# kisasexypantera94/hpfw

Hardware: AMD Instinct MI355X
Metric: hashprints/sec (index) + Hamming matches/sec (search), 30 s@44.1 kHz clips (higher is better)
Workload: dtype f32 (transforms, dB) + int8 digits / int64 sums (projection); 1 GPU; configs[1]: 1000 x 30 s synthetic 44.1 kHz PCM16 clips per GPU, hashprint extraction only (CQT + dB + projection + bit pack), inputs resident in HBM; clips_per_gpu=1000, hashprints_per_clip=2320, parallelism=clips sharded over 1 GPU(s), no collective on this path

## Files before the change

### hpfw_amd/csrc/k_forward.hip

```cpp
#include <cstdlib>

#include "kernels.h"

namespace hpfw {

extern __shared__ __align__(16) unsigned char smem_raw[];

typedef int v4i __attribute__((ext_vector_type(4)));
typedef int v16i __attribute__((ext_vector_type(16)));

constexpr int kCqThreads = 256;
constexpr int kCqCols = 128;
constexpr int kCqKSteps = 7;
constexpr int kCqKChunk = 32 * kCqKSteps;
constexpr int kCqTilesPerGroup = 7;
constexpr int kCqPlaneBytes = kCqCols * kCqKChunk;
constexpr int kCqABytes = kCqKSteps * 3 * 1024;
constexpr int kCqLdsBytes = 2 * kCqPlaneBytes + kCqABytes;

__device__ __forceinline__ int cq_slot(int c)
{
    const int l = c & 31;
    return (c & ~31) | (((l >> 2) ^ l) & 1) | (((l >> 3) & 1) << 1) | (((l >> 4) & 1) << 2) | (((l >> 1) & 1) << 3) | ((l & 1) << 4);
}
// ... 338 lines not shown
    cq3_load_samples<LOADW>(a, clip_pcm, col0 + wave * 32, sc, lane, x, [&] { issue_a(0, 0); });
    CQ_STAMP(0);
    const int c = col0 + wave * 32 + nl;
    const bool c_in = c < a.n2;
    const bool vec4 = (a.n2 & 3) == 0;
    static_assert(32 * kCq3Waves == kZBlock, "a workgroup's columns are one block of z");
    float *zblk = z + (int64_t)clip * a.zclip + (int64_t)cb * 2 * a.hq * kZBlock + wave * 32;
    const int rows_live = 2 * a.hq;
    double *corr_lds = reinterpret_cast<double *>(smem_raw + 2 * kCqABytes + kCq3Waves * kCq3ScratchBytes);
    for (int i = tid; i < kCq3CorrRows; i += 64 * kCq3Waves) corr_lds[i] = a.corr[i < rows_live ? i : rows_live - 1];
    for (int mt = 0; mt < a.mt; ++mt) {
        asm volatile("s_waitcnt vmcnt(0) lgkmcnt(0)\n\ts_barrier" ::: "memory");
        CQ_STAMP(1);
        const v4i *wb = reinterpret_cast<const v4i *>(abytes + (mt & 1) * kCqABytes) + lane;
        v16i acc[4];
        const v16i zero = v16i{0};
        auto step = [&](int s) {
            const v4i w0 = wb[(s * 3 + 0) * 64], w1 = wb[(s * 3 + 1) * 64], w2 = wb[(s * 3 + 2) * 64];
            acc[0] = __builtin_amdgcn_mfma_i32_32x32x32_i8(w0, x[s][0], s == 0 ? zero : acc[0], 0, 0, 0);
            acc[1] = __builtin_amdgcn_mfma_i32_32x32x32_i8(w1, x[s][0], s == 0 ? zero : acc[1], 0, 0, 0);
            acc[2] = __builtin_amdgcn_mfma_i32_32x32x32_i8(w2, x[s][0], s == 0 ? zero : acc[2], 0, 0, 0);
            acc[3] = __builtin_amdgcn_mfma_i32_32x32x32_i8(w2, x[s][1], s == 0 ? zero : acc[3], 0, 0, 0);
            acc[1] = __builtin_amdgcn_mfma_i32_32x32x32_i8(w0, x[s][1], acc[1], 0, 0, 0);
            acc[2] = __builtin_amdgcn_mfma_i32_32x32x32_i8(w1, x[s][1], acc[2], 0, 0, 0);
        };
        if (steps == kCqKSteps) {
#pragma unroll
            for (int s = 0; s < kCqKSteps; ++s) step(s);
        } else {
#pragma unroll
            for (int s = 0; s < kCqKSteps; ++s)
                if (s < steps) step(s);
        }
        CQ_STAMP(2);
        CQ_STAMP(3);
        if (mt + 1 < a.mt) issue_a(mt + 1, (mt + 1) & 1);
        asm volatile("" ::: "memory");
        CQ_STAMP(4);
        const int row0 = 32 * mt + 4 * h;
#pragma unroll
        for (int g = 0; g < 4; ++g) {
            float q[4];
#pragma unroll
            for (int e = 0; e < 4; ++e) {
                const int r = 4 * g + e;
                const int lo = acc[0][r] + (acc[1][r] << 8), hi = acc[2][r] + (acc[3][r] << 8);
                q[e] = (float)(__builtin_fma((double)hi, 65536.0, (double)lo) + corr_lds[row0 + 8 * g + e]);
            }
            if (vec4) {
#pragma unroll
                for (int pr = 0; pr < 2; ++pr) {
                    const float send = (lane & 1) ? q[2 * pr] : q[2 * pr + 1];
                    const float got = __builtin_bit_cast(float, __builtin_amdgcn_mov_dpp(__builtin_bit_cast(int, send), 0xB1, 0xF, 0xF, true));
                    if (lane & 1) q[2 * pr] = got; else q[2 * pr + 1] = got;
                }
#pragma unroll
                for (int pr = 0; pr < 2; ++pr) {
                    const float send = (lane & 2) ? q[pr] : q[pr + 2];
                    const float got = __builtin_bit_cast(float, __builtin_amdgcn_mov_dpp(__builtin_bit_cast(int, send), 0x4E, 0xF, 0xF, true));
                    if (lane & 2) q[pr] = got; else q[pr + 2] = got;
                }
                const int row = row0 + 8 * g + (nl & 3);
                const int c4 = col0 + wave * 32 + (nl & ~3);
                if (c4 < a.n2 && row < rows_live) *reinterpret_cast<float4 *>(zblk + row * kZBlock + (nl & ~3)) = float4{q[0], q[1], q[2], q[3]};
            } else {
#pragma unroll
                for (int e = 0; e < 4; ++e) {
                    const int row = row0 + 8 * g + e;
                    if (c_in && row < rows_live) zblk[row * kZBlock + nl] = q[e];
                }
            }
        }
        CQ_STAMP(6);
    }
#ifdef HPFW_COLS_STAMPS
    if (a.stamps && tid == 0) {
        long long *o = a.stamps + (int64_t)blockIdx.x * 8;
#pragma unroll
        for (int k = 0; k < 8; ++k) o[k] = st[k];
    }
#endif
}

#ifdef HPFW_COLS_STAMPS
long long *g_cols_stamps = nullptr;
extern "C" long long *hpfw_debug_cols_stamps() { return g_cols_stamps; }
#endif

constexpr int kFwdThreads = 512;
#ifndef HPFW_ROWS_WAVES
#define HPFW_ROWS_WAVES 6
#endif

template <class Groups, int WAVES>
__global__ __launch_bounds__(kFwdThreads, WAVES) void fwd_rows2_kernel(RowsArgs a, Rows2Out o, const float *__restrict__ z,
                                                                   cf *__restrict__ x)
{
    cf *lds = reinterpret_cast<cf *>(smem_raw);
    const int clip = blockIdx.x, q1 = blockIdx.y;
    rows2_body<Groups>(lds, a, kFwdThreads, z + (int64_t)clip * o.zclip + (int64_t)2 * q1 * o.zrow, q1, o, x + (int64_t)clip * o.n1 * o.q2w);
}

__global__ __launch_bounds__(256) void gather_bins_kernel(CqPlanDev cp, const cf *__restrict__ x, cf *__restrict__ out)
{
    const int clip = blockIdx.y;
    const XsView v = cp.view(x, clip);
    for (int i = blockIdx.x * 256 + threadIdx.x; i < cp.nk; i += gridDim.x * 256) out[(int64_t)clip * cp.nk + i] = v(cp.kmin + i);
}

template <int LOADW>
static void launch_cols_q_t(ColsQArgs a, const int16_t *d_pcm, int64_t clip_samples, dim3 grid, float *d_z, hipStream_t s)
{
    static PerDeviceOnce attr_set;
    if (attr_set.need()) {
        (void)hipFuncSetAttribute(reinterpret_cast<const void *>(fwd_cols_q_kernel<LOADW, true>), hipFuncAttributeMaxDynamicSharedMemorySize, kCqLdsBytes);
        (void)hipFuncSetAttribute(reinterpret_cast<const void *>(fwd_cols_q_kernel<LOADW, false>), hipFuncAttributeMaxDynamicSharedMemorySize, kCqLdsBytes);
        attr_set.mark();
    }
    if (a.ks <= kCqKSteps && !(a.variant & 1)) {
        a.n_clips = grid.x;
        constexpr int kWaves = 4;
        const int ncb = (a.n2 + 32 * kWaves - 1) / (32 * kWaves);
        hipLaunchKernelGGL((fwd_cols_q3_kernel<LOADW, kWaves>), dim3(8 * ((grid.x * ncb + 7) / 8)), dim3(64 * kWaves), cq3_lds_bytes(kWaves), s,
                           a, d_pcm, clip_samples, d_z);
        return;
    }
    if (a.n1 <= 255)
        hipLaunchKernelGGL((fwd_cols_q_kernel<LOADW, true>), grid, dim3(kCqThreads), kCqLdsBytes, s, a, d_pcm, clip_samples, d_z);
    else
        hipLaunchKernelGGL((fwd_cols_q_kernel<LOADW, false>), grid, dim3(kCqThreads), kCqLdsBytes, s, a, d_pcm, clip_samples, d_z);
}

void launch_fwd_cols_q(const ColsQArgs &a_in, const int16_t *d_pcm, int64_t clip_samples, int n_clips, float *d_z, hipStream_t s)
{
    if (n_clips <= 0) return;
    ColsQArgs a = a_in;
#ifdef HPFW_COLS_STAMPS
    static long long *d_stamps = nullptr;
    if (!d_stamps) (void)hipMalloc(&d_stamps, (size_t)64 * 1024 * 1024);
    a.stamps = d_stamps;
    g_cols_stamps = d_stamps;
#endif
    dim3 grid(n_clips, (a.n2 + kCqCols - 1) / kCqCols, (a.mt + kCqTilesPerGroup - 1) / kCqTilesPerGroup);
    const uintptr_t addr = reinterpret_cast<uintptr_t>(d_pcm);
    if (a.n2 % 4 == 0 && a.n2 >= 4 && addr % 8 == 0 && clip_samples % 4 == 0)
        launch_cols_q_t<4>(a, d_pcm, clip_samples, grid, d_z, s);
    else if (a.n2 % 2 == 0 && addr % 4 == 0 && clip_samples % 2 == 0)
        launch_cols_q_t<2>(a, d_pcm, clip_samples, grid, d_z, s);
    else
        launch_cols_q_t<1>(a, d_pcm, clip_samples, grid, d_z, s);
}

size_t fwd_rows_lds_bytes(const RowsArgs &a) { return (size_t)a.n2 * sizeof(cf); }

template <class Groups, int WAVES>
static void launch_rows2_t(const RowsArgs &a, const Rows2Out &o, const float *d_z, int n_clips, cf *d_x, hipStream_t s)
{
    static PerDeviceOnce attr_set;
    if (attr_set.need()) {
        (void)hipFuncSetAttribute(reinterpret_cast<const void *>(fwd_rows2_kernel<Groups, WAVES>),
                                  hipFuncAttributeMaxDynamicSharedMemorySize, 160 * 1024);
        attr_set.mark();
    }
    dim3 grid(n_clips, o.hq);
    hipLaunchKernelGGL((fwd_rows2_kernel<Groups, WAVES>), grid, dim3(kFwdThreads), fwd_rows_lds_bytes(a), s, a, o, d_z, d_x);
}

void launch_fwd_rows2(const RowsArgs &a, const Rows2Out &o, const float *d_z, int n_clips, cf *d_x, hipStream_t s)
{
    if (n_clips <= 0) return;
    if (Groups6300::matches_plan(a) && Groups6300::min_threads(a.n2) <= kFwdThreads)
        launch_rows2_t<Groups6300, HPFW_ROWS_WAVES>(a, o, d_z, n_clips, d_x, s);
    else
        launch_rows2_t<RuntimeGroups, 4>(a, o, d_z, n_clips, d_x, s);
}

void launch_gather_bins(const CqPlanDev &cp, const cf *d_x, int n_clips, cf *d_out, hipStream_t s)
{
    if (n_clips <= 0) return;
    hipLaunchKernelGGL(gather_bins_kernel, dim3((cp.nk + 255) / 256 < 64 ? (cp.nk + 255) / 256 : 64, n_clips), dim3(256), 0, s, cp, d_x, d_out);
}

}
```

### hpfw_amd/csrc/kernels.h

```cpp
#pragma once
#include <cmath>
#include <cstdint>
#include <vector>
#include <atomic>
#include <hip/hip_runtime.h>
#include <stdint.h>

#include "device_math.h"
#include "fft_lds.h"
#include "fft_rows.h"

namespace hpfw {

struct PerDeviceOnce {
    std::atomic<uint64_t> done{0};
    static uint64_t bit()
    {
        int dev = 0;
        (void)hipGetDevice(&dev);
        return 1ull << (dev & 63);
    }
    bool need() const { return !(done.load(std::memory_order_acquire) & bit()); }
    void mark() { done.fetch_or(bit(), std::memory_order_release); }
};


constexpr int kBins = 121;
constexpr int kCtx = 20;
constexpr int kLag = 80;
constexpr int kFilters = 64;
constexpr int kFrame = kBins * kCtx;

constexpr int kZBlock = 128;
inline long long z_floats_per_clip(int hq, int n2) { return (long long)((n2 + kZBlock - 1) / kZBlock) * 2 * hq * kZBlock; }

struct ColsQArgs {
    int n1, n2, hq;
    int mt, ks;
    const void *image;
    const double *corr;
    long long *stamps;
    int n_clips;
    int variant;
    long long zclip;
};

#ifndef HPFW_XS_BATCH
#define HPFW_XS_BATCH 4
#endif
constexpr int kXsBatch = HPFW_XS_BATCH;
struct XsView {
    const cf *base;
    int n1, w, q0;
    unsigned long long magic;
    HPFW_DEVICE_MEMBER cf operator()(int k) const
    {
        if (n1 == 1) return base[k - q0];
        const int q2 = (int)(((unsigned long long)(unsigned)k * magic) >> 40);
        return base[(int64_t)(k - q2 * n1) * w + (q2 - q0)];
    }
};
struct XsBand {
    XsView v;
    int start;
    HPFW_DEVICE_MEMBER cf operator()(int i) const { return v(start + i); }
    template <class F>
    HPFW_DEVICE_MEMBER void for_each(int tid, int nthreads, int lg, const cf *__restrict__ g, F f) const
    {
        for (int i0 = tid; i0 < lg; i0 += kXsBatch * nthreads) {
            cf xv[kXsBatch], gv[kXsBatch];
#pragma unroll
            for (int u = 0; u < kXsBatch; ++u) {
                const int i = i0 + u * nthreads;
                const int ic = i < lg ? i : lg - 1;
                xv[u] = v(start + ic);
                gv[u] = g[ic];
            }
#pragma unroll
            for (int u = 0; u < kXsBatch; ++u) {
                const int i = i0 + u * nthreads;
                if (i < lg) f(i, c_mul(xv[u], gv[u]));
            }
        }
    }
};
struct XsBandRows {
    const cf *base;
    int n1, w, q0;
    int start, q2a, nq2;
    unsigned magic;
    template <class F>
    HPFW_DEVICE_MEMBER void for_each(int tid, int nthreads, int lg, const cf *__restrict__ g2, F f) const
    {
        const int total = n1 * nq2;
        for (int t0 = tid; t0 < total; t0 += kXsBatch * nthreads) {
            cf xv[kXsBatch], gv[kXsBatch];
            int ii[kXsBatch];
#pragma unroll
            for (int u = 0; u < kXsBatch; ++u) {
                const int t = t0 + u * nthreads;
                const int tc = t < total ? t : total - 1;
                const int q1 = nq2 == 1 ? tc : (int)(((unsigned long long)(unsigned)tc * magic) >> 32);
                const int tq = tc - q1 * nq2;
                const int i = q1 + n1 * (q2a + tq) - start;
                ii[u] = (t < total && i >= 0 && i < lg) ? i : -1;
                xv[u] = base[(int64_t)q1 * w + (q2a - q0 + tq)];
                gv[u] = g2[tc];
            }
#pragma unroll
            for (int u = 0; u < kXsBatch; ++u)
                if (ii[u] >= 0) f(ii[u], c_mul(xv[u], gv[u]));
        }
    }
};

struct BzArgs {
    int n1, n2, n2pad;
    int kmin, kmax;
    int a;
    int n_tiles1;
    int k1lo, k1n;
    int n_tiles2;
    int nt2;
    const float *wp;
    const cf *tl;
    const cf *bhat;
// ... 167 lines not shown
```

### hpfw_amd/csrc/plan.cpp

```cpp
#include "plan.h"
#include "trig_d.h"

#include <algorithm>
#include <atomic>
#include <cmath>
#include <cstring>
#include <map>
#include <memory>
#include <mutex>
#include <thread>

namespace hpfw {

namespace {
constexpr double kSampleRate = 44100.0;
constexpr double kMinFreq = 130.81;
constexpr double kMaxFreq = 4186.01;
constexpr int kBpo = 24;
constexpr int kMinWindow = 96;
constexpr int kDown = 3;
constexpr int kBins = 121;
constexpr int kCtx = 20;
constexpr int kLag = 80;
constexpr int64_t kN2Max = 6826;
// ... 309 lines not shown
    }
    const int64_t n2 = p.bluestein ? 6300 : n / n1;
    std::vector<int> tmp;
    std::vector<int> desc;
    if (!make_radix_list(n2, desc) || (!p.bluestein && !make_radix_list(n1, tmp))) {
        why = "clip length has a prime factor other than 2, 3, 5, 7";
        return false;
    }
    for (size_t lo = 0, hi = desc.size(); lo < hi;) {
        p.radix.push_back(desc[lo++]);
        if (lo < hi) p.radix.push_back(desc[--hi]);
    }
    if (n1 > 8192) {
        why = "clip too long";
        return false;
    }
    p.n1 = (int)n1;
    p.n2 = (int)n2;
    p.h = (int)(n2 / 2 + 1);
    p.k1lo = (int)(kmin / n2);
    p.k1hi = (int)((kmax - 1) / n2);
    if (geometry_only) return true;
    p.tw_n2 = twiddle_table(n2);
    p.tw_n1 = twiddle_table(n1);
    for (size_t i = 0; i < p.radix.size();) {
        if (i + 1 < p.radix.size() && p.radix[i] * p.radix[i + 1] <= 36) {
            p.groups.push_back({p.radix[i], p.radix[i + 1]});
            i += 2;
        } else {
            p.groups.push_back({p.radix[i], 1});
            i += 1;
        }
    }
    if (p.groups.size() > 12) {
        why = "too many radix passes";
        return false;
    }
    {
        int64_t len = n2;
        for (const auto &g : p.groups) {
            p.rows_gtw_off.push_back((int)p.rows_gtw.size());
            append_group_twiddles(p.tw_n2, n2, len, g.first, g.second, p.rows_gtw);
            len /= g.first * g.second;
        }
    }
    if (!p.bluestein) {
        const int64_t hq = n1 / 2 + 1;
        p.hq = (int)hq;
        p.q2lo = (int)(kmin / n1);
        p.q2w = (int)((kmax - 1) / n1) - p.q2lo + 1;
        p.cols_mt = (int)((2 * hq + 31) / 32);
        p.cols_ks = (int)((n1 + 31) / 32);
        p.wq.resize((size_t)2 * n1);
        for (int64_t m = 0; m < n1; ++m) {
            double c, s;
            twiddle_d(m, n1, c, s);
            p.wq[(size_t)(2 * m)] = (int32_t)std::rint(c * 4194304.0);
            p.wq[(size_t)(2 * m + 1)] = (int32_t)std::rint(s * 4194304.0);
        }
        p.cols_corr.assign((size_t)2 * hq, 0.0);
        for (int64_t q1 = 0; q1 < hq; ++q1) {
            int64_t sr = 0, si = 0;
            for (int64_t k1 = 0; k1 < n1; ++k1) {
                sr += p.wq[(size_t)(2 * ((q1 * k1) % n1))];
                si += p.wq[(size_t)(2 * ((q1 * k1) % n1) + 1)];
            }
            p.cols_corr[(size_t)(2 * q1)] = (double)(128 * sr);
            p.cols_corr[(size_t)(2 * q1 + 1)] = (double)(128 * si);
        }
        p.cols_image.assign((size_t)p.cols_mt * p.cols_ks * 3 * 1024, 0);
        parallel_rows(p.cols_mt, [&](int64_t mt) {
            for (int64_t ks = 0; ks < p.cols_ks; ++ks)
                for (int l = 0; l < 64; ++l)
                    for (int e = 0; e < 16; ++e) {
                        const int64_t row = 32 * mt + (l & 31), k1 = 32 * ks + 16 * (l >> 5) + e, q1 = row >> 1;
                        if (q1 >= hq || k1 >= n1) continue;
                        const int w = p.wq[(size_t)(2 * ((q1 * k1) % n1) + (row & 1))];
                        const int d0 = ((w + 128) & 255) - 128, w1 = (w - d0) >> 8, d1 = ((w1 + 128) & 255) - 128, d2 = (w1 - d1) >> 8;
                        const int d[3] = {d0, d1, d2};
                        for (int i = 0; i < 3; ++i)
                            p.cols_image[((((size_t)mt * p.cols_ks + ks) * 3 + i) * 64 + l) * 16 + e] = (int8_t)d[i];
                    }
        });
        const int64_t nq = (n2 + 3) / 4;
        p.ts_seed.resize((size_t)(hq * nq));
        p.ts_step.resize((size_t)(hq * 4));
        parallel_rows(hq, [&](int64_t q1) {
            for (int64_t m = 0; m < nq; ++m) {
                const HostCf t = twiddle_f((q1 * 4 * m) % n, n);
                p.ts_seed[(size_t)(q1 * nq + m)] = {std::ldexp(t.r, -37), std::ldexp(t.i, -37)};
            }
            p.ts_step[(size_t)(q1 * 4)] = {1.0f, 0.0f};
            for (int e = 1; e < 4; ++e) p.ts_step[(size_t)(q1 * 4 + e)] = twiddle_f((q1 * e) % n, n);
        });
    }
    p.pos_n2.resize((size_t)n2);
    for (int64_t k = 0; k < n2; ++k) p.pos_n2[(size_t)k] = (int)digit_pos(k, n2, p.radix);
    {
        const int r1 = p.groups.back().first, r2 = p.groups.back().second, len = r1 * r2;
        const int nb = (int)(n2 / len);
        p.kb_last.assign((size_t)nb, -1);
        for (int k = 0; k < nb; ++k) p.kb_last[(size_t)(p.pos_n2[(size_t)k] / len)] = k;
        for (int b = 0; b < nb; ++b)
            for (int s = 0; s < r1; ++s)
                for (int s2 = 0; s2 < r2; ++s2)
                    if (p.kb_last[(size_t)b] < 0 ||
                        p.pos_n2[(size_t)(p.kb_last[(size_t)b] + nb * (s + r1 * s2))] != len * b + s * r2 + s2) {
                        why = "internal: last-group output map";
                        return false;
                    }
    }
    p.g_off.assign(kBins, 0);
    int64_t goff = 0;
    for (int j = 0; j < kBins; ++j) {
        const int64_t need = p.lg[j] + p.c - 1;
        const int64_t ps = chirpz_length(need);
        if (ps > (1 << 19)) {
            why = "clip too long: chirp-z length above 2^19";
            return false;
        }
        p.psize[j] = (int)ps;
        size_t k = 0;
        for (; k < p.classes.size(); ++k)
            if (p.classes[k].p == ps) break;
        if (k == p.classes.size()) {
            BluesteinClass bc;
            bc.p = (int)ps;
            p.classes.push_back(std::move(bc));
        }
        p.classes[k].bands.push_back(j);
        p.g_off[j] = goff;
        goff += p.lg[j];
    }
    std::atomic<bool> bad_class{false};
    parallel_rows((int64_t)p.classes.size(), [&](int64_t ci) {
        BluesteinClass &bc = p.classes[(size_t)ci];
        const int64_t ps = bc.p;
        make_radix_list(ps, bc.radix);
        bc.tw = twiddle_table(ps);
        {
            auto next_radix = [](int64_t len) { return len % 4 == 0 ? 4 : (len % 3 == 0 ? 3 : 2); };
            int64_t len = ps;
            while (ps > 16384 && len > 8192) {
                len /= 4;
                ++bc.outer;
            }
            bc.len0 = (int)len;
            int g = 0;
            for (;;) {
                const int r1 = next_radix(len);
                const int r2 = len / r1 > 1 ? next_radix(len / r1) : 1;
                const int64_t rest = len / (r1 * r2);
                if (rest == 1) {
                    std::vector<HostCf> tmp;
                    append_group_twiddles(bc.tw, ps, len, r1, r2, tmp);
                    bc.mid_off = (int)bc.gtw.size();
                    for (int e = 0; e < (r1 - 1) * r2; ++e) bc.gtw.push_back(tmp[(size_t)e]);
                    break;
                }
                if (g >= 4) {
                    bad_class = true;
                    return;
                }
                bc.goff[g++] = (int)bc.gtw.size();
                append_group_twiddles(bc.tw, ps, len, r1, r2, bc.gtw);
                len /= r1 * r2;
// ... 195 lines not shown
```

### hpfw_amd/csrc/plan.h

```cpp
#pragma once
#include <cstdint>
#include <string>
#include <utility>
#include <vector>

namespace hpfw {

struct HostCf {
    float r, i;
};

struct BluesteinClass {
    int p = 0;
    std::vector<int> radix;
    std::vector<HostCf> tw;
    std::vector<HostCf> gtw;
    int goff[4] = {0, 0, 0, 0};
    int mid_off = 0;
    std::vector<HostCf> vrev;
    std::vector<int> bands;
    int len0 = 0, outer = 0;
};

struct HostPlan {
    int64_t n = 0;
    int n1 = 0, n2 = 0, h = 0;
    int kmin = 0, kmax = 0, k1lo = 0, k1hi = 0;
    int m = 0, c = 0, n_frames = 0, n_hp = 0;
    std::vector<int> radix;
    std::vector<std::pair<int, int>> groups;
    std::vector<HostCf> rows_gtw;
    std::vector<int> rows_gtw_off;
    std::vector<HostCf> tw_n2, tw_n1;
    std::vector<HostCf> tw_big;
    int hq = 0;
    int q2lo = 0, q2w = 0;
    int cols_mt = 0, cols_ks = 0;
    std::vector<int32_t> wq;
    std::vector<int8_t> cols_image;
    std::vector<double> cols_corr;
    std::vector<HostCf> ts_seed;
    std::vector<HostCf> ts_step;
    std::vector<int> pos_n2;
    std::vector<int> kb_last;
    int start[121], lg[121], psize[121];
    std::vector<int64_t> g_off;
    int64_t g_total = 0, big_m = 0;
    std::vector<HostCf> g;
    std::vector<BluesteinClass> classes;
    bool bluestein = false;
    int64_t bz_l = 0;
};

enum : unsigned {
    kConvHannPeriodic = 1u,
    kConvLgHalfEven = 2u,
    kConvFloatGeometry = 4u,
    kConvNoIfftScale = 8u,
    kConvAll = 15u
};
struct PlanSerial {
    PlanSerial();
    ~PlanSerial();
    bool before;
};
bool build_plan(int64_t n_samples, HostPlan &out, std::string &why, bool geometry_only = false,
                bool force_bluestein = false, unsigned conventions = 0, bool host_windows = true);
inline double cq_window_scale(unsigned conventions, int64_t big_m, int psize)
{
    return 1.0 / (((conventions & kConvNoIfftScale) ? 1.0 : (double)big_m) * (double)psize);
}
inline int64_t cq_hann_den(unsigned conventions, int64_t lg) { return (conventions & kConvHannPeriodic) ? lg : lg - 1; }

bool build_frame_transform(int n2, HostPlan &out, std::string &why);
void mel_tables(std::vector<float> &window, std::vector<float> &cpack);

void twiddle_d(int64_t m, int64_t n, double &re, double &im);
int64_t digit_pos(int64_t k, int64_t n, const std::vector<int> &radix);
bool make_radix_list(int64_t n, std::vector<int> &radix);
void append_group_twiddles(const std::vector<HostCf> &tw, int64_t n, int64_t len, int r1, int r2,
                           std::vector<HostCf> &out);

}
```

### hpfw_amd/csrc/plans.hip

```cpp
#include "handle.h"

struct PlanTiming {
    double host_wait = 0, host_build = 0, upload = 0, device_tables = 0, alloc = 0, evict = 0, total = 0;
    long plans = 0, copies = 0;
    size_t copied = 0;
};

namespace {
thread_local size_t g_uploaded = 0;

hpfw::RadixList to_radix(const std::vector<int> &r)
{
    hpfw::RadixList rl;
    std::memset(&rl, 0, sizeof(rl));
    rl.n = (int)r.size();
    for (size_t i = 0; i < r.size(); ++i) rl.r[i] = r[i];
    return rl;
}

DevBuf pool_take(hpfw_gpu *h, size_t bytes);
void pool_give(hpfw_gpu *h, DevBuf b);
void pool_release(hpfw_gpu *h);

constexpr size_t kPlanChunk = (size_t)4 << 20;
// ... 212 lines not shown
    std::memset(&bz, 0, sizeof(bz));
    if (p.bluestein) {
        PlanTimer t_dev(&PlanTiming::device_tables);
        bz.n1 = p.n1;
        bz.n2 = p.n2;
        bz.n2pad = (p.n2 + 31) / 32 * 32;
        bz.kmin = p.kmin;
        bz.kmax = p.kmax;
        bz.a = p.n1 / 16;
        bz.n_tiles1 = (bz.a + 15) / 16;
        bz.k1lo = p.kmin / p.n2;
        bz.k1n = (p.kmax - 1) / p.n2 - bz.k1lo + 1;
        {
            const int need = (2 * bz.k1n + 31) / 32;
            bz.nt2 = need < 3 ? need : 3;
            bz.n_tiles2 = (need + bz.nt2 - 1) / bz.nt2 * bz.nt2;
        }
        const cf *d_tw_n1 = nullptr;
        struct PoolTmp {
            hpfw_gpu *h;
            std::vector<DevBuf> v;
            ~PoolTmp() { for (DevBuf &b : v) pool_give(h, std::move(b)); }
            void *take(size_t bytes)
            {
                DevBuf b = pool_take(h, (bytes + 65535) / 65536 * 65536);
                if (!b) return nullptr;
                v.push_back(std::move(b));
                return v.back().get();
            }
        } tmp{h, {}};
        {
            void *d = tmp.take(p.tw_n1.size() * sizeof(cf));
            if (!d) return fail(HPFW_E_HIP, "out of device memory for the tables of a clip length");
            HIP_TRY(plan_h2d(h, d, p.tw_n1.data(), p.tw_n1.size() * sizeof(cf)));
            d_tw_n1 = static_cast<const cf *>(d);
        }
        {
            const size_t bytes[3] = {(size_t)bz.a * bz.n_tiles1 * 64 * sizeof(float), (size_t)bz.a * 16 * 64 * sizeof(float),
                                     (size_t)p.n1 * bz.n_tiles2 * 64 * sizeof(float)};
            const float **slot[3] = {&bz.apack1, &bz.apack3, &bz.apack2};
            for (int i = 0; i < 3; ++i) {
                void *d = nullptr;
                if ((rc = plan_alloc(dp.get(), bytes[i], &d))) return rc;
                g_uploaded += bytes[i];
                *slot[i] = static_cast<const float *>(d);
            }
            if ((rc = plan_flush(dp.get()))) return rc;
            hpfw::launch_bz_pack_stages(bz, d_tw_n1, const_cast<float *>(bz.apack1), const_cast<float *>(bz.apack3), h->cache.plan_stream.get());
            hpfw::launch_bz_pack_coefficients(p.n1, bz.k1lo, bz.k1n, d_tw_n1, bz.n_tiles2, const_cast<float *>(bz.apack2), h->cache.plan_stream.get());
        }
        const size_t big_l = (size_t)p.n1 * p.n2, plane = hpfw::bz_plane_bytes(bz, 1);
        {
            const size_t bytes[4] = {big_l * sizeof(cf), big_l * sizeof(cf), big_l * sizeof(cf), (size_t)(p.kmax - p.kmin) * sizeof(cf)};
            const void **slot[4] = {reinterpret_cast<const void **>(&bz.wp), reinterpret_cast<const void **>(&bz.tl),
                                    reinterpret_cast<const void **>(&bz.bhat), reinterpret_cast<const void **>(&bz.wk)};
            for (int i = 0; i < 4; ++i) {
                void *d = nullptr;
                if ((rc = plan_alloc(dp.get(), bytes[i], &d))) return rc;
                g_uploaded += bytes[i];
                *slot[i] = d;
            }
        }
        void *scratch = tmp.take(big_l * 8 + plane);
        if (!scratch) return fail(HPFW_E_HIP, "out of device memory for the tables of a clip length");
        hpfw::launch_bz_make_tables(ra, bz, n, static_cast<float *>(scratch), static_cast<float *>(scratch) + 2 * big_l, h->cache.plan_stream.get());
        const hipError_t launched = hipGetLastError();
        if (launched != hipSuccess) return fail(HPFW_E_HIP, std::string("chirp-z tables: ") + hipGetErrorString(launched));
    }
    hpfw::ColsQArgs &ca = dp->cols;
    std::memset(&ca, 0, sizeof(ca));
    dp->rows_out = hpfw::Rows2Out{p.n1, p.hq, p.q2lo, p.q2w, nullptr, nullptr, (p.n2 + 3) / 4, 5 ,
                                  (long long)2 * p.hq * hpfw::kZBlock, hpfw::kZBlock, hpfw::z_floats_per_clip(p.hq, p.n2)};
    static_assert(hpfw::kZBlock == 128, "Rows2Out::zshift4 above");
    if (!p.bluestein) {
        ca.n1 = p.n1;
        ca.n2 = p.n2;
        ca.hq = p.hq;
        ca.mt = p.cols_mt;
        ca.ks = p.cols_ks;
        ca.zclip = hpfw::z_floats_per_clip(p.hq, p.n2);
        const int8_t *img = nullptr;
        if ((rc = upload(p.cols_image, &img, dp.get()))) return rc;
        ca.image = img;
        if ((rc = upload(p.cols_corr, &ca.corr, dp.get()))) return rc;
        if ((rc = upload(p.ts_seed, reinterpret_cast<const hpfw::HostCf **>(&dp->rows_out.seed), dp.get()))) return rc;
        if ((rc = upload(p.ts_step, reinterpret_cast<const hpfw::HostCf **>(&dp->rows_out.step), dp.get()))) return rc;
    }
    hpfw::CqPlanDev &c = dp->cq;
    c.kmin = p.kmin;
    c.nk = p.kmax - p.kmin;
    c.c = p.c;
    if (p.bluestein) {
        c.xn1 = 1;
        c.xw = 0;
        c.xq0 = p.kmin;
        c.xclip = c.nk;
        c.xmagic = 0;
    } else {
        c.xn1 = p.n1;
        c.xw = p.q2w;
        c.xq0 = p.q2lo;
        c.xclip = (int64_t)p.n1 * p.q2w;
        c.xmagic = ((1ull << 40) + (unsigned long long)p.n1 - 1) / (unsigned long long)p.n1;
    }
    std::vector<int> start(p.start, p.start + 121), lg(p.lg, p.lg + 121);
    if ((rc = upload(start, &c.start, dp.get()))) return rc;
    if ((rc = upload(lg, &c.lg, dp.get()))) return rc;
    if ((rc = upload(p.g_off, &c.g_off, dp.get()))) return rc;
    {
        void *d = nullptr;
        if ((rc = plan_alloc(dp.get(), (size_t)std::max<int64_t>(p.g_total, 1) * sizeof(cf), &d))) return rc;
        g_uploaded += (size_t)p.g_total * sizeof(cf);
        c.g = static_cast<const cf *>(d);
    }
    int g2_max_entries = 0;
    c.g2 = nullptr;
    c.g2_off = nullptr;
    c.q2a = c.nq2 = nullptr;
    c.nq2_magic = nullptr;
    c.rows_min = 4;
    if (!p.bluestein) {
        std::vector<int> q2a(121), nq2(121);
        std::vector<unsigned> magic(121);
        std::vector<int64_t> g2_off(121);
        int64_t total = 0;
        for (int j = 0; j < 121; ++j) {
            q2a[j] = p.start[j] / p.n1;
            nq2[j] = (p.start[j] + p.lg[j] - 1) / p.n1 - q2a[j] + 1;
            magic[j] = nq2[j] >= 2 ? (unsigned)(((1ull << 32) + (unsigned)nq2[j] - 1) / (unsigned)nq2[j]) : 0u;
            g2_off[j] = total;
            total += (int64_t)p.n1 * nq2[j];
        }
        for (int j = 0; j < 121; ++j) g2_max_entries = std::max(g2_max_entries, p.n1 * nq2[j]);
        {
            void *d = nullptr;
            if ((rc = plan_alloc(dp.get(), (size_t)std::max<int64_t>(total, 1) * sizeof(cf), &d))) return rc;
            g_uploaded += (size_t)total * sizeof(cf);
            c.g2 = static_cast<const cf *>(d);
        }
        if ((rc = upload(g2_off, &c.g2_off, dp.get()))) return rc;
        if ((rc = upload(q2a, &c.q2a, dp.get()))) return rc;
        if ((rc = upload(nq2, &c.nq2, dp.get()))) return rc;
        if ((rc = upload(magic, &c.nq2_magic, dp.get()))) return rc;
    }
    for (const hpfw::BluesteinClass &bc : p.classes) {
        hpfw::CqClassDev cd;
        cd.p = bc.p;
        cd.n_bands = (int)bc.bands.size();
        cd.radix = to_radix(bc.radix);
        if ((rc = upload(bc.tw, reinterpret_cast<const hpfw::HostCf **>(&cd.tw), dp.get()))) return rc;
        if ((rc = upload(bc.gtw, reinterpret_cast<const hpfw::HostCf **>(&cd.gtw.tab), dp.get()))) return rc;
        for (int g = 0; g < 4; ++g) cd.gtw.off[g] = bc.goff[g];
        cd.gtw.mid_off = bc.mid_off;
        if ((rc = upload(bc.vrev, reinterpret_cast<const hpfw::HostCf **>(&cd.vrev), dp.get()))) return rc;
        if ((rc = upload(bc.bands, &cd.band, dp.get()))) return rc;
        cd.len0 = bc.len0;
        cd.outer = bc.outer;
        dp->cls.push_back(cd);
    }
    if ((size_t)p.n2 * sizeof(cf) > 150 * 1024) return fail(HPFW_E_UNSUPPORTED, "n2 exceeds the LDS");
    {
        hpfw::HostPlan &hp = dp->hp;
        std::vector<hpfw::HostCf>().swap(hp.rows_gtw);
        std::vector<hpfw::HostCf>().swap(hp.tw_n2);
        std::vector<hpfw::HostCf>().swap(hp.tw_n1);
        std::vector<hpfw::HostCf>().swap(hp.ts_seed);
        std::vector<int8_t>().swap(hp.cols_image);
        std::vector<hpfw::HostCf>().swap(hp.g);
        for (hpfw::BluesteinClass &bc : hp.classes) {
            std::vector<hpfw::HostCf>().swap(bc.tw);
            std::vector<hpfw::HostCf>().swap(bc.gtw);
            std::vector<hpfw::HostCf>().swap(bc.vrev);
        }
    }
    dp->bytes = g_uploaded;
    dp->last_use = ++h->cache.plan_clock;
    size_t budget = (size_t)16 << 30;
    if (const char *e = std::getenv("HPFW_PLAN_CACHE_GB")) budget = (size_t)(std::max(0.0, std::atof(e)) * 1073741824.0);
    if (h->cache.plan_bytes + dp->bytes > budget && !h->cache.plans.empty()) {
        PlanTimer t(&PlanTiming::evict);
        size_t goal = budget;
        while (h->cache.plan_bytes + dp->bytes > goal && !h->cache.plans.empty()) {
            auto lru = h->cache.plans.begin();
            for (auto q = h->cache.plans.begin(); q != h->cache.plans.end(); ++q)
                if (q->second->last_use < lru->second->last_use) lru = q;
            if (lru->second->last_use > h->cache.idle_clock) {
                HIP_TRY(hipDeviceSynchronize());
                h->cache.idle_clock = h->cache.plan_clock;
                goal = budget - budget / 4;
            }
            h->cache.plan_bytes -= lru->second->bytes;
            {
                std::scoped_lock lock(h->cache.host_mtx);
                h->cache.host_seen.erase(lru->first);
            }
            h->cache.plans.erase(lru);
        }
    }
    if ((rc = plan_flush(dp.get()))) return rc;
    std::vector<char>().swap(dp->stage);
    {
        PlanTimer t(&PlanTiming::device_tables);
        hpfw::CqWindowBands wb;
        int lg_max = 0;
        for (int j = 0; j < 121; ++j) {
            wb.scale[j] = hpfw::cq_window_scale(h->conventions, p.big_m, p.psize[j]);
            wb.hann_den[j] = (int)hpfw::cq_hann_den(h->conventions, p.lg[j]);
            lg_max = std::max(lg_max, p.lg[j]);
        }
        hpfw::launch_cq_windows(c, wb, p.big_m, lg_max, const_cast<cf *>(c.g), h->cache.plan_stream.get());
        if (c.g2) hpfw::launch_cq_windows_rows(c, p.n1, g2_max_entries, const_cast<cf *>(c.g2), h->cache.plan_stream.get());
        const hipError_t launched = hipGetLastError();
        if (launched != hipSuccess) return fail(HPFW_E_HIP, std::string("constant-Q window tables: ") + hipGetErrorString(launched));
    }
    HIP_TRY(hipEventRecord(h->cache.plan_ev.get(), h->cache.plan_stream.get()));
    h->cache.plan_ev_pending = true;
    h->cache.plan_bytes += dp->bytes;
    *out = dp.get();
    h->cache.plans[n] = std::move(dp);
    return 0;
}

hipError_t init_plans(hpfw_gpu *h)
{
    if (std::getenv("HPFW_PLAN_TIMING")) h->cache.plan_timing = std::make_unique<PlanTiming>();
    const hipError_t e = h->cache.plan_ev.create();
    return e != hipSuccess ? e : h->cache.plan_stream.create();
}

void clear_plans(hpfw_gpu *h)
{
    h->cache.plans.clear();
    h->cache.plan_bytes = 0;
    std::unique_lock<std::mutex> lock(h->cache.host_mtx);
    h->cache.host_cv.wait(lock, [&] {
        for (auto &kv : h->cache.host_ready)
            if (!kv.second) return false;
        return true;
    });
    h->cache.host_ready.clear();
    h->cache.host_seen.clear();
}

hpfw_gpu::PlanCache::PlanCache() = default;
hpfw_gpu::PlanCache::~PlanCache()
{
    if (!plan_timing || !plan_timing->plans) return;
    const PlanTiming &t = *plan_timing;
    std::fprintf(stderr, "hpfw plan timing: %ld lengths, %.1f ms in get_plan = %.3f ms each: wait for the host half %.3f, host build %.3f, "
                         "uploads %.3f (%ld copies, %.2f MB per length), device tables (incl. their uploads) %.3f, device memory %.3f, "
// ... 103 lines not shown
```

Measured before the change: 247.9 million hashprints/s.

## Add symmetry-folded int8 MFMA column DFT kernel using half-period twiddle structure

Result: faster. 263.2 million hashprints/s, median of 6 (+6.2%).

```diff
diff --git a/hpfw_amd/csrc/k_forward.hip b/hpfw_amd/csrc/k_forward.hip
--- a/hpfw_amd/csrc/k_forward.hip
+++ b/hpfw_amd/csrc/k_forward.hip
@@ -444,6 +444,262 @@
 #endif
 }
 
+constexpr int kCq4Steps = 2;
+constexpr int kCq4ABytes = 2 * kCq4Steps * 3 * 1024;
+constexpr int kCq4ScratchBytes = 2 * 4 * 32 * 16;
+constexpr int cq4_lds_bytes(int waves) { return 2 * kCq4ABytes + waves * kCq4ScratchBytes + kCq3CorrRows * 8; }
+
+__device__ __forceinline__ int cq4_slot(int c)
+{
+    return ((c >> 2) & 1) | (((c >> 3) & 1) << 1) | ((((c >> 4) ^ (c >> 1)) & 1) << 2) | ((c & 1) << 3) | (((c >> 1) & 1) << 4);
+}
+
+__device__ __forceinline__ void cq4_store_pair(unsigned char *sc, int c, int rq, unsigned r0, unsigned r1, unsigned r2, unsigned r3)
+{
+    const unsigned x01 = __builtin_amdgcn_perm(r1, r0, 0x05010400u), x23 = __builtin_amdgcn_perm(r3, r2, 0x05010400u);
+    const unsigned y01 = __builtin_amdgcn_perm(r1, r0, 0x07030602u), y23 = __builtin_amdgcn_perm(r3, r2, 0x07030602u);
+    const int a0 = (rq >> 2) * 512 + cq4_slot(c) * 16 + 4 * (rq & 3), a1 = (rq >> 2) * 512 + cq4_slot(c + 1) * 16 + 4 * (rq & 3);
+    *reinterpret_cast<unsigned *>(sc + a0) = __builtin_amdgcn_perm(x23, x01, 0x05040100u);
+    *reinterpret_cast<unsigned *>(sc + 2048 + a0) = __builtin_amdgcn_perm(x23, x01, 0x07060302u);
+    *reinterpret_cast<unsigned *>(sc + a1) = __builtin_amdgcn_perm(y23, y01, 0x05040100u);
+    *reinterpret_cast<unsigned *>(sc + 2048 + a1) = __builtin_amdgcn_perm(y23, y01, 0x07060302u);
+}
+
+template <int LOADW, class F>
+__device__ __forceinline__ void cq4_load_samples(const ColsQArgs &a, const int16_t *__restrict__ clip_pcm, int cw0,
+                                                 unsigned char *sc, int lane, v4i (&x)[2 * kCq4Steps][2][2], F issued)
+{
+    const int cg = lane & 7, quad = lane >> 3;
+    const int row_last = a.n1 - 1, last = a.n2 - 1;
+    const int gc = cw0 + 4 * cg;
+    const char *base = reinterpret_cast<const char *>(clip_pcm);
+    const unsigned pitch = 2u * (unsigned)a.n2;
+    unsigned cb[4];
+    if (LOADW == 4) {
+        cb[0] = 2u * (unsigned)(gc + 3 <= last ? gc : last - 3);
+    } else if (LOADW == 2) {
+        cb[0] = 2u * (unsigned)(gc + 1 <= last ? gc : last - 1);
+        cb[1] = 2u * (unsigned)(gc + 3 <= last ? gc + 2 : last - 1);
+    } else {
+#pragma unroll
+        for (int e = 0; e < 4; ++e) cb[e] = 2u * (unsigned)(gc + e <= last ? gc + e : last);
+    }
+    constexpr int kItems = 2 * kCq4Steps;
+    constexpr int kBatch = LOADW == 4 ? kItems : 1;
+    const int rd0 = (lane >> 4) * 512 + cq4_slot(lane & 15) * 16, rd1 = (lane >> 4) * 512 + cq4_slot(16 + (lane & 15)) * 16;
+#pragma unroll
+    for (int i0 = 0; i0 < kItems; i0 += kBatch) {
+    unsigned r[kBatch][8][2];
+#pragma unroll
+    for (int ib = 0; ib < kBatch; ++ib) {
+        const int par = (i0 + ib) / kCq4Steps, s = (i0 + ib) % kCq4Steps;
+#pragma unroll
+        for (int i = 0; i < 8; ++i) {
+            int row = 2 * (64 * s + 32 * (i >> 2) + 4 * quad + (i & 3)) + par;
+            if (row > row_last) row = row_last;
+            const unsigned ro = (unsigned)row * pitch;
+            if (LOADW == 4) {
+                const uint2 v = *reinterpret_cast<const uint2 *>(base + (ro + cb[0]));
+                r[ib][i][0] = v.x;
+                r[ib][i][1] = v.y;
+            } else if (LOADW == 2) {
+                r[ib][i][0] = *reinterpret_cast<const unsigned *>(base + (ro + cb[0]));
+                r[ib][i][1] = *reinterpret_cast<const unsigned *>(base + (ro + cb[1]));
+            } else {
+                r[ib][i][0] = (unsigned)*reinterpret_cast<const unsigned short *>(base + (ro + cb[0])) |
+                              ((unsigned)*reinterpret_cast<const unsigned short *>(base + (ro + cb[1])) << 16);
+                r[ib][i][1] = (unsigned)*reinterpret_cast<const unsigned short *>(base + (ro + cb[2])) |
+                              ((unsigned)*reinterpret_cast<const unsigned short *>(base + (ro + cb[3])) << 16);
+            }
+        }
+    }
+    if (i0 == 0) issued();
+#pragma unroll
+    for (int ib = 0; ib < kBatch; ++ib) {
+#pragma unroll
+        for (int i = 0; i < 8; ++i) {
+            r[ib][i][0] ^= 0x00800080u;
+            r[ib][i][1] ^= 0x00800080u;
+        }
+#pragma unroll
+        for (int hf = 0; hf < 2; ++hf) {
+            cq4_store_pair(sc, 4 * cg, 8 * hf + quad, r[ib][4 * hf][0], r[ib][4 * hf + 1][0], r[ib][4 * hf + 2][0], r[ib][4 * hf + 3][0]);
+            cq4_store_pair(sc, 4 * cg + 2, 8 * hf + quad, r[ib][4 * hf][1], r[ib][4 * hf + 1][1], r[ib][4 * hf + 2][1], r[ib][4 * hf + 3][1]);
+        }
+        asm volatile("s_waitcnt lgkmcnt(0)" ::: "memory");
+        x[i0 + ib][0][0] = *reinterpret_cast<const v4i *>(sc + rd0);
+        x[i0 + ib][0][1] = *reinterpret_cast<const v4i *>(sc + 2048 + rd0);
+        x[i0 + ib][1][0] = *reinterpret_cast<const v4i *>(sc + rd1);
+        x[i0 + ib][1][1] = *reinterpret_cast<const v4i *>(sc + 2048 + rd1);
+        asm volatile("s_waitcnt lgkmcnt(0)" ::: "memory");
+    }
+    }
+}
+
+__device__ __forceinline__ void cq4_quad_transpose(float (&q)[4], int lane)
+{
+#pragma unroll
+    for (int pr = 0; pr < 2; ++pr) {
+        const float send = (lane & 1) ? q[2 * pr] : q[2 * pr + 1];
+        const float got = __builtin_bit_cast(float, __builtin_amdgcn_mov_dpp(__builtin_bit_cast(int, send), 0xB1, 0xF, 0xF, true));
+        if (lane & 1) q[2 * pr] = got; else q[2 * pr + 1] = got;
+    }
+#pragma unroll
+    for (int pr = 0; pr < 2; ++pr) {
+        const float send = (lane & 2) ? q[pr] : q[pr + 2];
+        const float got = __builtin_bit_cast(float, __builtin_amdgcn_mov_dpp(__builtin_bit_cast(int, send), 0x4E, 0xF, 0xF, true));
+        if (lane & 2) q[pr] = got; else q[pr + 2] = got;
+    }
+}
+
+template <int LOADW, int kCq4Waves>
+__global__ __launch_bounds__(64 * kCq4Waves, 3) void fwd_cols_q4_kernel(ColsQArgs a, const int16_t *__restrict__ pcm, int64_t clip_samples,
+                                                                    float *__restrict__ z)
+{
+    constexpr int kCq4Cols = 32 * kCq4Waves;
+    unsigned char *abytes = smem_raw;
+    const int tid = threadIdx.x, lane = tid & 63, wave = tid >> 6;
+    unsigned char *sc = smem_raw + 2 * kCq4ABytes + wave * kCq4ScratchBytes;
+    const int ncb = (a.n2 + kCq4Cols - 1) / kCq4Cols;
+    const unsigned per_xcd = (gridDim.x + 7) / 8;
+    const unsigned t = (blockIdx.x & 7) * per_xcd + (blockIdx.x >> 3);
+    if (t >= (unsigned)(a.n_clips * ncb)) return;
+    const int cb = t % ncb, clip = t / ncb;
+    const int col0 = cb * kCq4Cols;
+    const int16_t *clip_pcm = pcm + (int64_t)clip * clip_samples;
+    const v4i *image = static_cast<const v4i *>(a.image2);
+    const int ks2 = a.ks2, pieces = 3 * 2 * ks2;
+    auto issue_a = [&](int mt, int buf) {
+        const v4i *src = image + (int64_t)mt * pieces * 64 + lane;
+#pragma unroll
+        for (int e = 0; e < (2 * kCq4Steps * 3 + kCq4Waves - 1) / kCq4Waves; ++e) {
+            const int p = wave + kCq4Waves * e;
+            if (p < pieces)
+                __builtin_amdgcn_global_load_lds((const __attribute__((address_space(1))) void *)(src + p * 64),
+                                                 (__attribute__((address_space(3))) void *)(abytes + buf * kCq4ABytes + p * 1024),
+                                                 16, 0, 0);
+        }
+    };
+#ifdef HPFW_COLS_STAMPS
+    long long st[8] = {0, 0, 0, 0, 0, 0, 0, 0};
+    long long tprev = __builtin_amdgcn_s_memtime();
+    auto stamp = [&](int k) {
+        const long long t = __builtin_amdgcn_s_memtime();
+        st[k] += t - tprev;
+        tprev = t;
+    };
+#endif
+    v4i x[2 * kCq4Steps][2][2];
+    cq4_load_samples<LOADW>(a, clip_pcm, col0 + wave * 32, sc, lane, x, [&] { issue_a(0, 0); });
+    CQ_STAMP(0);
+    const int u = lane >> 4, nl = lane & 15;
+    const int hh = a.n1 >> 1, q1_last = hh >> 1;
+    const bool vec4 = (a.n2 & 3) == 0;
+    static_assert(32 * kCq4Waves == kZBlock, "a workgroup's columns are one block of z");
+    float *zblk = z + (int64_t)clip * a.zclip + (int64_t)cb * 2 * a.hq * kZBlock + wave * 32;
+    const int rows_live = 2 * a.hq;
+    double *corr_lds = reinterpret_cast<double *>(smem_raw + 2 * kCq4ABytes + kCq4Waves * kCq4ScratchBytes);
+    for (int i = tid; i < kCq3CorrRows; i += 64 * kCq4Waves) corr_lds[i] = a.corr[i < rows_live ? i : rows_live - 1];
+    for (int mt = 0; mt < a.mt2; ++mt) {
+        asm volatile("s_waitcnt vmcnt(0) lgkmcnt(0)\n\ts_barrier" ::: "memory");
+        CQ_STAMP(1);
+        const v4i *wb = reinterpret_cast<const v4i *>(abytes + (mt & 1) * kCq4ABytes) + lane;
+        const v4i zero = v4i{0, 0, 0, 0};
+        v4i lo[2][2], hi[2][2];
+#pragma unroll
+        for (int par = 0; par < 2; ++par) {
+            v4i acc[4][2];
+#pragma unroll
+            for (int s = 0; s < kCq4Steps; ++s) {
+                if (s == 0 || s < ks2) {
+                    const v4i *w = wb + (par * ks2 + s) * 3 * 64;
+                    const v4i w0 = w[0], w1 = w[64], w2 = w[128];
+                    const v4i(&xs)[2][2] = x[par * kCq4Steps + s];
+#pragma unroll
+                    for (int ct = 0; ct < 2; ++ct) {
+                        acc[0][ct] = __builtin_amdgcn_mfma_i32_16x16x64_i8(w0, xs[ct][0], s == 0 ? zero : acc[0][ct], 0, 0, 0);
+                        acc[1][ct] = __builtin_amdgcn_mfma_i32_16x16x64_i8(w1, xs[ct][0], s == 0 ? zero : acc[1][ct], 0, 0, 0);
+                        acc[2][ct] = __builtin_amdgcn_mfma_i32_16x16x64_i8(w2, xs[ct][0], s == 0 ? zero : acc[2][ct], 0, 0, 0);
+                        acc[3][ct] = __builtin_amdgcn_mfma_i32_16x16x64_i8(w2, xs[ct][1], s == 0 ? zero : acc[3][ct], 0, 0, 0);
+                    }
+#pragma unroll
+                    for (int ct = 0; ct < 2; ++ct) {
+                        acc[1][ct] = __builtin_amdgcn_mfma_i32_16x16x64_i8(w0, xs[ct][1], acc[1][ct], 0, 0, 0);
+                        acc[2][ct] = __builtin_amdgcn_mfma_i32_16x16x64_i8(w1, xs[ct][1], acc[2][ct], 0, 0, 0);
+                    }
+                }
+            }
+#pragma unroll
+            for (int ct = 0; ct < 2; ++ct) {
+                lo[par][ct] = acc[0][ct] + (acc[1][ct] << 8);
+                hi[par][ct] = acc[2][ct] + (acc[3][ct] << 8);
+            }
+        }
+        CQ_STAMP(2);
+        if (mt + 1 < a.mt2) issue_a(mt + 1, (mt + 1) & 1);
+        asm volatile("" ::: "memory");
+        CQ_STAMP(4);
+        const int q1a = 8 * mt + 2 * u;
+        const double *cp = corr_lds + 16 * mt + 4 * u;
+        const double *cm0 = corr_lds + 2 * max(hh - q1a, 0), *cm1 = corr_lds + 2 * max(hh - q1a - 1, 0);
+        float gp[2][4], gm[2][4];
+#pragma unroll
+        for (int ct = 0; ct < 2; ++ct)
+#pragma unroll
+            for (int r = 0; r < 4; ++r) {
+                const int el = lo[0][ct][r], eh = hi[0][ct][r], ol = lo[1][ct][r], oh = hi[1][ct][r];
+                gp[ct][r] = (float)(__builtin_fma((double)(eh + oh), 65536.0, (double)(el + ol)) + cp[r]);
+                const int ml = (r & 1) ? ol - el : el - ol, mh = (r & 1) ? oh - eh : eh - oh;
+                gm[ct][r] = (float)(__builtin_fma((double)mh, 65536.0, (double)ml) + (r < 2 ? cm0 : cm1)[r & 1]);
+            }
+        if (vec4) {
+            const int j = lane & 3, col = 16 * (u >> 1) + (nl & ~3);
+            const bool c_ok = col0 + wave * 32 + col < a.n2;
+#pragma unroll
+            for (int sgn = 0; sgn < 2; ++sgn) {
+                float(&g)[2][4] = sgn ? gm : gp;
+                cq4_quad_transpose(g[0], lane);
+                cq4_quad_transpose(g[1], lane);
+                float sa[4], sb[4];
+#pragma unroll
+                for (int e = 0; e < 4; ++e) {
+                    const auto sw = __builtin_amdgcn_permlane32_swap(__builtin_bit_cast(unsigned, g[0][e]), __builtin_bit_cast(unsigned, g[1][e]), false, false);
+                    sa[e] = __builtin_bit_cast(float, (unsigned)sw[0]);
+                    sb[e] = __builtin_bit_cast(float, (unsigned)sw[1]);
+                }
+#pragma unroll
+                for (int half = 0; half < 2; ++half) {
+                    const int tr = 8 * half + 4 * (u & 1) + j, q1 = 8 * mt + (tr >> 1);
+                    const int row = sgn ? 2 * (hh - q1) + (tr & 1) : 16 * mt + tr;
+                    const bool live = q1 <= q1_last && (!sgn || 2 * q1 < hh);
+                    const float(&s4)[4] = half ? sb : sa;
+                    if (c_ok && live) *reinterpret_cast<float4 *>(zblk + row * kZBlock + col) = float4{s4[0], s4[1], s4[2], s4[3]};
+                }
+            }
+        } else {
+            const int c = col0 + wave * 32 + nl;
+#pragma unroll
+            for (int ct = 0; ct < 2; ++ct)
+#pragma unroll
+                for (int r = 0; r < 4; ++r) {
+                    const int q1 = q1a + (r >> 1);
+                    if (c + 16 * ct < a.n2 && q1 <= q1_last) {
+                        zblk[(2 * q1 + (r & 1)) * kZBlock + 16 * ct + nl] = gp[ct][r];
+                        if (2 * q1 < hh) zblk[(2 * (hh - q1) + (r & 1)) * kZBlock + 16 * ct + nl] = gm[ct][r];
+                    }
+                }
+        }
+        CQ_STAMP(6);
+    }
+#ifdef HPFW_COLS_STAMPS
+    if (a.stamps && tid == 0) {
+        long long *o = a.stamps + (int64_t)blockIdx.x * 8;
+#pragma unroll
+        for (int k = 0; k < 8; ++k) o[k] = st[k];
+    }
+#endif
+}
+
 #ifdef HPFW_COLS_STAMPS
 long long *g_cols_stamps = nullptr;
 extern "C" long long *hpfw_debug_cols_stamps() { return g_cols_stamps; }
@@ -483,6 +739,11 @@
         a.n_clips = grid.x;
         constexpr int kWaves = 4;
         const int ncb = (a.n2 + 32 * kWaves - 1) / (32 * kWaves);
+        if (a.image2 && !(a.variant & 2)) {
+            hipLaunchKernelGGL((fwd_cols_q4_kernel<LOADW, kWaves>), dim3(8 * ((grid.x * ncb + 7) / 8)), dim3(64 * kWaves), cq4_lds_bytes(kWaves), s,
+                               a, d_pcm, clip_samples, d_z);
+            return;
+        }
         hipLaunchKernelGGL((fwd_cols_q3_kernel<LOADW, kWaves>), dim3(8 * ((grid.x * ncb + 7) / 8)), dim3(64 * kWaves), cq3_lds_bytes(kWaves), s,
                            a, d_pcm, clip_samples, d_z);
         return;
diff --git a/hpfw_amd/csrc/kernels.h b/hpfw_amd/csrc/kernels.h
--- a/hpfw_amd/csrc/kernels.h
+++ b/hpfw_amd/csrc/kernels.h
@@ -42,6 +42,8 @@
     long long *stamps;
     int n_clips;
     int variant;
+    int mt2, ks2;
+    const void *image2;
     long long zclip;
 };
 
diff --git a/hpfw_amd/csrc/plan.cpp b/hpfw_amd/csrc/plan.cpp
--- a/hpfw_amd/csrc/plan.cpp
+++ b/hpfw_amd/csrc/plan.cpp
@@ -415,6 +415,34 @@
                             p.cols_image[((((size_t)mt * p.cols_ks + ks) * 3 + i) * 64 + l) * 16 + e] = (int8_t)d[i];
                     }
         });
+        if (n1 % 2 == 0 && p.cols_ks <= 7) {
+            const int64_t h = n1 / 2;
+            bool symmetric = true;
+            for (int64_t m = 0; m < n1 && symmetric; ++m) {
+                const int32_t *w = &p.wq[(size_t)(2 * m)], *wh = &p.wq[(size_t)(2 * ((m + h) % n1))], *wc = &p.wq[(size_t)(2 * ((n1 - m) % n1))];
+                symmetric = wh[0] == -w[0] && wh[1] == -w[1] && wc[0] == w[0] && wc[1] == -w[1];
+            }
+            if (symmetric) {
+                const int64_t nq1 = h / 2 + 1;
+                p.cols2_mt = (int)((2 * nq1 + 15) / 16);
+                p.cols2_ks = (int)((h + 63) / 64);
+                p.cols2_image.assign((size_t)p.cols2_mt * 2 * p.cols2_ks * 3 * 1024, 0);
+                parallel_rows(p.cols2_mt, [&](int64_t mt) {
+                    for (int64_t st = 0; st < 2 * p.cols2_ks; ++st)
+                        for (int l = 0; l < 64; ++l)
+                            for (int e = 0; e < 16; ++e) {
+                                const int64_t row = 16 * mt + (l & 15), q1 = row >> 1, par = st / p.cols2_ks;
+                                const int64_t m = 64 * (st % p.cols2_ks) + 16 * (l >> 4) + e, k1 = 2 * m + par;
+                                if (q1 >= nq1 || m >= h) continue;
+                                const int w = p.wq[(size_t)(2 * ((q1 * k1) % n1) + (row & 1))];
+                                const int d0 = ((w + 128) & 255) - 128, w1 = (w - d0) >> 8, d1 = ((w1 + 128) & 255) - 128, d2 = (w1 - d1) >> 8;
+                                const int d[3] = {d0, d1, d2};
+                                for (int i = 0; i < 3; ++i)
+                                    p.cols2_image[((((size_t)mt * 2 * p.cols2_ks + st) * 3 + i) * 64 + l) * 16 + e] = (int8_t)d[i];
+                            }
+                });
+            }
+        }
         const int64_t nq = (n2 + 3) / 4;
         p.ts_seed.resize((size_t)(hq * nq));
         p.ts_step.resize((size_t)(hq * 4));
diff --git a/hpfw_amd/csrc/plan.h b/hpfw_amd/csrc/plan.h
--- a/hpfw_amd/csrc/plan.h
+++ b/hpfw_amd/csrc/plan.h
@@ -39,6 +39,8 @@
     std::vector<int32_t> wq;
     std::vector<int8_t> cols_image;
     std::vector<double> cols_corr;
+    int cols2_mt = 0, cols2_ks = 0;
+    std::vector<int8_t> cols2_image;
     std::vector<HostCf> ts_seed;
     std::vector<HostCf> ts_step;
     std::vector<int> pos_n2;
diff --git a/hpfw_amd/csrc/plans.hip b/hpfw_amd/csrc/plans.hip
--- a/hpfw_amd/csrc/plans.hip
+++ b/hpfw_amd/csrc/plans.hip
@@ -318,6 +318,12 @@
         const int8_t *img = nullptr;
         if ((rc = upload(p.cols_image, &img, dp.get()))) return rc;
         ca.image = img;
+        if (!p.cols2_image.empty()) {
+            ca.mt2 = p.cols2_mt;
+            ca.ks2 = p.cols2_ks;
+            if ((rc = upload(p.cols2_image, &img, dp.get()))) return rc;
+            ca.image2 = img;
+        }
         if ((rc = upload(p.cols_corr, &ca.corr, dp.get()))) return rc;
         if ((rc = upload(p.ts_seed, reinterpret_cast<const hpfw::HostCf **>(&dp->rows_out.seed), dp.get()))) return rc;
         if ((rc = upload(p.ts_step, reinterpret_cast<const hpfw::HostCf **>(&dp->rows_out.step), dp.get()))) return rc;
@@ -402,6 +408,7 @@
         std::vector<hpfw::HostCf>().swap(hp.tw_n1);
         std::vector<hpfw::HostCf>().swap(hp.ts_seed);
         std::vector<int8_t>().swap(hp.cols_image);
+        std::vector<int8_t>().swap(hp.cols2_image);
         std::vector<hpfw::HostCf>().swap(hp.g);
         for (hpfw::BluesteinClass &bc : hp.classes) {
             std::vector<hpfw::HostCf>().swap(bc.tw);
```
